# XiandaGuo/OpenStereo

Measured on NVIDIA H100. Metric: stereo_pairs_per_sec_gwcnet_256x512_d192, higher is better.
Workload: dtype f32

## Files before the change

### include/openstereo_b200.h

```cpp
#ifndef OPENSTEREO_B200_H_
#define OPENSTEREO_B200_H_

#include <stddef.h>
#include <stdint.h>

#ifdef __cplusplus
extern "C" {
#endif

#define OSB_OK 0
#define OSB_EINVAL 1
#define OSB_ECUDA 2
#define OSB_EUNSUPPORTED 3

#define OSB_ACT_NONE 0
#define OSB_ACT_RELU 1
#define OSB_ACT_LEAKY 2
#define OSB_ACT_RELU6 3

typedef void* osb_stream_t;

int osb_abi_version(void);
const char* osb_last_error(void);
uint64_t osb_launch_count(void);
// ... 85 lines not shown
                            osb_stream_t stream);
int osb_conv3d_k3_s2_tc_cs_fwd(const float* x_ndhwc, const void* w_split, const float* scale, const float* shift, float* y, int B,
                               int Cin, int Cout, int D, int H, int W, int act, int ystride, osb_stream_t stream);
int osb_deconv3d_k4_tc_cs_fwd(const float* x_ndhwc, const void* w_split, const float* scale, const float* shift, float* y, int B,
                              int Cin, int Cout, int D, int H, int W, int act, int ystride, osb_stream_t stream);
int osb_conv1x1_ndhwc_cat_fwd(const float* x0, const float* x1, int C0, int C1, const float* w_packed, const float* scale,
                              const float* shift, float* y, long long voxels, int Cout, int act, osb_stream_t stream);
int osb_conv1x1_ndhwc_fwd(const float* x, const float* w_packed, const float* scale, const float* shift, float* y,
                          long long voxels, int Cin, int Cout, int act, osb_stream_t stream);
int osb_conv3d_k3_c1_ndhwc_fwd(const float* x_ndhwc, const float* w_taps, const float* scale, const float* shift, float* y, int B,
                               int Cin, int D, int H, int W, osb_stream_t stream);
int osb_conv2d_tc_kc(int Cin, int Cout, int W, int dilation);
int osb_conv2d_k3_tc_fwd(const float* x_nhwc, const void* w_split, const float* scale, const float* shift, const float* residual,
                         float* y, int B, int Cin, int Cout, int H, int W, int dilation, int act, int out_nhwc, int res_nhwc,
                         osb_stream_t stream);
int osb_gwc_volume_sum_fwd(const float* ref, const float* tgt, float* out, int B, int C, int H, int W, int D, int G,
                           osb_stream_t stream);
int osb_group_l2_normalize_fwd(const float* x, float* y, int B, int C, int H, int W, int G, float eps, osb_stream_t stream);
int osb_sub_volume_fwd(const float* left, const float* right, float* out, int B, int C, int H, int W, int D, osb_stream_t stream);
int osb_regression_values_fwd(const float* prob, const float* values, float* out, int B, int D, int H, int W, osb_stream_t stream);

int osb_warped_concat_volume_fwd(const float* x, const float* y, const float* disp, float* out, int B, int C, int D, int H, int W,
                                 int mask_left, osb_stream_t stream);
int osb_warped_gwc_concat_volume_fwd(const float* xg, const float* yg, const float* xc, const float* yc, const float* disp,
                                     float* out, int B, int Cg, int G, int Cc, int D, int H, int W, osb_stream_t stream);

int osb_coex_regression_fwd(const float* cost, const float* spx, float* out, int B, int D, int h, int w, int top_k, int spx_is_logits,
                            osb_stream_t stream);
int osb_nearest_resize3d_fwd(const float* x, float* y, int N, int Di, int Hi, int Wi, int Do, int Ho, int Wo, osb_stream_t stream);

// ... 34 lines not shown
```

### openstereo_b200/_lib.py

```python
import ctypes
import os

_PKG = os.path.dirname(os.path.abspath(__file__))
LIB_PATH = os.path.join(_PKG, "lib", "libopenstereo_b200.so")

_f32p = ctypes.c_void_p
_i = ctypes.c_int
_f = ctypes.c_float
_s = ctypes.c_void_p

SIGNATURES = {
    "osb_gwc_volume_fwd": [_f32p, _f32p, _f32p, _i, _i, _i, _i, _i, _i, _s],
    "osb_concat_volume_fwd": [_f32p, _f32p, _f32p, _i, _i, _i, _i, _i, _i, _s],
    "osb_gwc_concat_volume_fwd": [_f32p, _f32p, _f32p, _f32p, _f32p, _i, _i, _i, _i, _i, _i, _i, _s],
    "osb_corr_volume_fwd": [_f32p, _f32p, _f32p, _i, _i, _i, _i, _i, _s],
    "osb_softargmin_fwd": [_f32p, _f32p, _i, _i, _i, _i, _f, _f, _f, _i, _s],
    "osb_upsample_softargmin_fwd": [_f32p, _f32p, _i, _i, _i, _i, _i, _i, _i, _i, _s],
    "osb_epe_partial_fwd": [_f32p, _f32p, _f32p, _i, _i, _f, _s],
    "osb_conv3d_k3_bn_act_fwd": [_f32p] * 7 + [_i] * 8 + [_s],
    "osb_deconv3d_bn_act_fwd": [_f32p] * 6 + [_i] * 8 + [_s],
    "osb_conv3d_1x1_bn_act_fwd": [_f32p, _f32p, _i] + [_f32p] * 6 + [_i] * 8 + [_s],
    "osb_conv3d_tc_supported": [_i, _i, _i, _i],
    "osb_conv3d_tc_kc": [_i, _i, _i, _i],
    "osb_tc_general_width": [_i],
# ... 9 lines not shown
    "osb_deconv3d_k4_tc_supported": [_i, _i, _i],
    "osb_conv3d_k3_tc_cs_fwd": [_f32p] * 7 + [_i] * 8 + [_s],
    "osb_conv3d_k3_s2_tc_cs_fwd": [_f32p] * 5 + [_i] * 8 + [_s],
    "osb_deconv3d_k4_tc_cs_fwd": [_f32p] * 5 + [_i] * 8 + [_s],
    "osb_deconv3d_k4_tc_fwd": [_f32p] * 6 + [_i] * 10 + [_s],
    "osb_conv1x1_ndhwc_cat_fwd": [_f32p, _f32p, _i, _i, _f32p, _f32p, _f32p, _f32p, ctypes.c_longlong, _i, _i, _s],
    "osb_feature_att_gate_fwd": [_f32p] * 8 + [_i] * 7 + [_s],
    "osb_ncdhw_to_ndhwc_pad": [_f32p, _f32p, _i, _i, _i, _i, _i, _i, _s],
    "osb_conv1x1_ndhwc_fwd": [_f32p] * 5 + [ctypes.c_longlong, _i, _i, _i, _s],
    "osb_conv3d_k3_c1_ndhwc_fwd": [_f32p] * 5 + [_i] * 5 + [_s],
    "osb_avgpool_pairs_fwd": [_f32p, _f32p, ctypes.c_longlong, _i, ctypes.c_longlong, _s],
    "osb_geo_lookup_fwd": [_f32p] * 11 + [_i] * 8 + [_s],
    "osb_context_upsample_fwd": [_f32p] * 3 + [_i] * 4 + [_s],
    "osb_conv2d_tc_kc": [_i] * 4,
    "osb_conv2d_k3_tc_fwd": [_f32p] * 6 + [_i] * 9 + [_s],
    "osb_ncdhw_to_ndhwc": [_f32p, _f32p, _i, _i, _i, _i, _i, _s],
    "osb_gwc_volume_sum_fwd": [_f32p, _f32p, _f32p, _i, _i, _i, _i, _i, _i, _s],
    "osb_group_l2_normalize_fwd": [_f32p, _f32p, _i, _i, _i, _i, _i, _f, _s],
    "osb_sub_volume_fwd": [_f32p, _f32p, _f32p, _i, _i, _i, _i, _i, _s],
    "osb_regression_values_fwd": [_f32p, _f32p, _f32p, _i, _i, _i, _i, _s],
    "osb_gwc_volume_bwd": [_f32p] * 5 + [_i] * 7 + [_s],
    "osb_concat_volume_bwd": [_f32p] * 3 + [_i] * 6 + [_s],
    "osb_softargmin_bwd": [_f32p] * 3 + [_i] * 4 + [_f, _f, _f, _i, _s],
    "osb_dwconv2d_fwd": [_f32p] * 6 + [_i] * 8 + [_s],
    "osb_deconv2d_k3s2_fwd": [_f32p] * 6 + [_i] * 6 + [_s],
    "osb_upsample_softargmin_values_fwd": [_f32p] * 3 + [_i] * 8 + [_s],
    "osb_warped_concat_volume_fwd": [_f32p] * 4 + [_i] * 6 + [_s],
    "osb_warped_gwc_concat_volume_fwd": [_f32p] * 6 + [_i] * 7 + [_s],
    "osb_coex_regression_fwd": [_f32p] * 3 + [_i] * 6 + [_s],
    "osb_nearest_resize3d_fwd": [_f32p] * 2 + [_i] * 7 + [_s],
# ... 58 lines not shown
```

### openstereo_b200/csrc/conv3d_tc.cu

```cuda
#include <type_traits>

#include "tc_common.cuh"

namespace osb {

constexpr int TC_W = 128;
constexpr int TC_KC = 32;
constexpr int TC_TILES = TC_WGS;
constexpr int TC_ROWS = TC_TILES + 2;
constexpr int TC_STAGES = 4;
constexpr int TC_RAW = 2;
constexpr int TC_ROW_BYTES = TC_W * TC_KC * 4;

struct TcParams {
  CUtensorMap xmap;
  const float* x;
  const void* w;
  const float* scale;
  const float* shift;
  const float* residual;
  float* y;
  int B, D, H, Cin, Cout;
  int act;
  float kappa;
// ... 402 lines not shown
  unsigned int* flag = tc_overflow_flag();
  if (!flag) return OSB_ECUDA;
  const size_t vol = (size_t)D * H * W;
  dim3 grid((unsigned)((vol + 31) / 32), (C + 31) / 32, B);
  ncdhw_to_ndhwc_kernel<<<grid, 256, 0, (cudaStream_t)stream>>>(x, nullptr, C, C, vol, reinterpret_cast<uint16_t*>(y_split), flag);
  count_launch();
  return check_launch("ncdhw_to_ndhwc_kernel");
}

int osb_ncdhw_to_ndhwc(const float* x, float* y, int B, int C, int D, int H, int W, osb_stream_t stream) {
  return osb_ncdhw_to_ndhwc_pad(x, y, B, C, C, D, H, W, stream);
}

static int conv3d_k3_tc_impl(osb::TcArgs a, int dilation, osb_stream_t stream) {
  using namespace osb;
  const int kc = select_conv3d_tc(a.Cin, a.Cout, a.W, dilation, false, false).kc;
  OSB_REQUIRE(kc, "conv3d_k3_tc: unsupported shape Cin=%d Cout=%d W=%d dilation=%d", a.Cin, a.Cout, a.W, dilation);
  OSB_REQUIRE(!a.in_ncdhw || kc == 32, "conv3d_k3_tc: NCDHW input is served by the W = 128 kernel only");
  OSB_REQUIRE((!a.ystride && !a.gate) || kc == 16, "conv3d_k3_tc: a channel slice or gate needs the 16-channel-chunk kernels");
  OSB_REQUIRE(a.Cout > 16 || (!a.out_ndhwc && (!a.residual || !a.res_ndhwc)), "conv3d_k3_tc: Cout <= 16 writes (and adds) NCDHW tensors only");
  OSB_REQUIRE(!(a.in_split || a.out_split || a.res_split) || (kc == 32 && !a.ystride && !a.gate),
              "conv3d_k3_tc: split activations are served by the W = 128 kernel only");
  OSB_REQUIRE(!a.in_split || !a.in_ncdhw, "conv3d_k3_tc: an input is either NCDHW or split");
  OSB_REQUIRE((!a.out_split || a.out_ndhwc) && (!a.res_split || a.res_ndhwc), "conv3d_k3_tc: split tensors are channels-last");
  OSB_REQUIRE(!(a.out_split || a.res_split) || (a.out_ndhwc && (!a.residual || a.res_ndhwc)),
              "conv3d_k3_tc: a split output or residual needs a channels-last output and residual");
  const TcLaunch launch = select_conv3d_tc(a.Cin, a.Cout, a.W, dilation, a.gate != nullptr, a.slice()).launch;
  const int rc = check_tc_args("conv3d_k3_tc", a, launch);
  return rc != OSB_OK ? rc : launch(a, (cudaStream_t)stream);
}

int osb_conv3d_k3_tc_fwd(const float* x_ndhwc, const void* w_split, const float* scale, const float* shift,
                         const float* residual, float* y, int B, int Cin, int Cout, int D, int H, int W, int act,
                         int out_ndhwc, int res_ndhwc, osb_stream_t stream) {
  return conv3d_k3_tc_impl({x_ndhwc, w_split, scale, shift, residual, nullptr, y, B, Cin, Cout, D, H, W, act, out_ndhwc, res_ndhwc, 0, 0,
                            Cout}, 1, stream);
}

int osb_conv3d_k3_tc_gate_fwd(const float* x_ndhwc, const void* w_split, const float* scale, const float* shift,
                              const float* residual, const float* gate_nhwc, float* y, int B, int Cin, int Cout, int D, int H, int W,
                              int act, osb_stream_t stream) {
// ... 4 lines not shown

int osb_conv3d_k3_tc_cs_fwd(const float* x_ndhwc, const void* w_split, const float* scale, const float* shift, const float* residual,
                            const float* gate_nhwc, float* y, int B, int Cin, int Cout, int D, int H, int W, int act, int ystride,
                            osb_stream_t stream) {
  return conv3d_k3_tc_impl({x_ndhwc, w_split, scale, shift, residual, gate_nhwc, y, B, Cin, Cout, D, H, W, act, 1, 1, 0, ystride, Cout},
                           1, stream);
}

int osb_conv3d_k3_tc_ncdhw_fwd(const float* x_ncdhw, const void* w_split, const float* scale, const float* shift,
                               const float* residual, float* y, int B, int Cin, int Cout, int D, int H, int W, int act,
                               int out_ndhwc, int res_ndhwc, osb_stream_t stream) {
  return conv3d_k3_tc_impl({x_ncdhw, w_split, scale, shift, residual, nullptr, y, B, Cin, Cout, D, H, W, act, out_ndhwc, res_ndhwc, 1, 0,
                            Cout}, 1, stream);
}

int osb_conv3d_k3_tc_split_fwd(const float* x, const void* w_split, const float* scale, const float* shift, const float* residual,
                               float* y, int B, int Cin, int Cout, int D, int H, int W, int act, int in_layout, int out_layout,
                               int res_layout, osb_stream_t stream) {
  auto known = [](int l) { return l == OSB_LAYOUT_NCDHW || l == OSB_LAYOUT_NDHWC || l == OSB_LAYOUT_SPLIT; };
  OSB_REQUIRE(known(in_layout) && known(out_layout) && known(res_layout), "conv3d_k3_tc_split: unknown layout");
  osb::TcArgs a{x, w_split, scale, shift, residual, nullptr, y, B, Cin, Cout, D, H, W, act, out_layout != OSB_LAYOUT_NCDHW, res_layout != OSB_LAYOUT_NCDHW,
                in_layout == OSB_LAYOUT_NCDHW, 0, Cout};
  a.in_split = in_layout == OSB_LAYOUT_SPLIT, a.out_split = out_layout == OSB_LAYOUT_SPLIT, a.res_split = res_layout == OSB_LAYOUT_SPLIT;
  return conv3d_k3_tc_impl(a, 1, stream);
}

int osb_conv2d_tc_kc(int Cin, int Cout, int W, int dilation) { return osb::select_conv3d_tc(Cin, Cout, W, dilation, false, false).kc; }

int osb_conv2d_k3_tc_fwd(const float* x_nhwc, const void* w_split, const float* scale, const float* shift, const float* residual,
                         float* y, int B, int Cin, int Cout, int H, int W, int dilation, int act, int out_nhwc, int res_nhwc,
                         osb_stream_t stream) {
  return conv3d_k3_tc_impl({x_nhwc, w_split, scale, shift, residual, nullptr, y, B, Cin, Cout, 1, H, W, act, out_nhwc, res_nhwc, 0, 0,
                            Cout}, dilation, stream);
}
}
```

### openstereo_b200/csrc/conv3d_tcg.cu

```cuda
#include "tc_common.cuh"

namespace osb {

struct TcgParams {
  const float* x;
  const void* w;
  const float* scale;
  const float* shift;
  const float* residual;
  const float* gate;
  float* y;
  int B, D, H, Cin;
  int act;
  float kappa;
  unsigned int* overflow;
  int out_ndhwc, res_ndhwc;
  int items, hblocks;
  int Wr, ctiles;
  int ystride;
};

template <int COUT, int KC, int W, int TILES, int DIL = 1, bool GW = false>
struct TcgCfg {
  static_assert(!GW || W == 128, "general-width tiles are 128-column segments of one image row");
  static constexpr int HALO = GW ? DIL : 0;
  static constexpr int CSTEP = 128 - 2 * HALO;
  static_assert(DIL == 1 || (W == 128 && DIL == 2 && COUT >= 64), "dilation 2 is instantiated for full-width rows only");
  static constexpr int R = 128 / W;
  static constexpr int ROWB = KC * 4;
  static constexpr int UNIT_BYTES = 128 * ROWB;
  static constexpr int N3 = 3 * COUT;
  static constexpr int G = 32;
  static constexpr int NG = COUT / G;
  static constexpr int NG3 = 3 * G;
  static constexpr int B_SLICE = N3 * ROWB;
  static constexpr int B_SUB = NG3 * ROWB;
  static constexpr int NT = TC_WGS * TILES;
  static constexpr int TS = R * DIL;
  static constexpr int HSPAN = NT * TS;
  __host__ __device__ static constexpr int row0(int hb) { return (hb / DIL) * HSPAN + (hb % DIL) * R; }
  __host__ static int hblocks(int H) { return DIL * ((H + HSPAN - 1) / HSPAN); }
  static constexpr int NLW = 4;
  static constexpr int XCHG_FLOATS = 2 * frag_xchg_floats<G, DIL>();
// ... 25 lines not shown
    return n;
  }
  static constexpr int NU = units_per_phase();
  static constexpr int unit_s(int j) {
    int k = 0;
    for (int s = S_FIRST; s <= S_LAST; ++s)
      if (used(s)) {
        if (k == j) return s;
        ++k;
      }
    return S_LAST;
  }
};

template <int COUT, int KC, int W, int TILES, int DIL = 1, bool GW = false, bool GATE = false>
__global__ void __launch_bounds__(TcgCfg<COUT, KC, W, TILES, DIL, GW>::THREADS, 1) conv3d_tcg_kernel(const TcgParams p) {
  using C = TcgCfg<COUT, KC, W, TILES, DIL, GW>;
  extern __shared__ __align__(1024) uint8_t smem_raw[];
  uint8_t* smem = reinterpret_cast<uint8_t*>((reinterpret_cast<uintptr_t>(smem_raw) + 1023) & ~static_cast<uintptr_t>(1023));
  uint8_t* a_buf = smem + C::A_OFF;
  uint8_t* b_buf = smem + C::B_OFF;
  uint64_t* bars = reinterpret_cast<uint64_t*>(smem + C::BAR_OFF);
  uint64_t* a_ready = bars;
  uint64_t* a_empty = a_ready + C::STAGES;
  uint64_t* b_full = a_empty + C::STAGES;
  uint64_t* b_empty = b_full + TC_BSLOTS * 3;
  float* xchg = reinterpret_cast<float*>(smem + C::BAR_OFF + 1024);
  float* tiles = xchg + TC_WGS * C::XCHG_FLOATS;
  float* s_scale = tiles + 4 * TC_WGS * FRAG_TP_FLOATS;
  float* s_shift = s_scale + COUT;

  const int warp = threadIdx.x >> 5, lane = threadIdx.x & 31;
  const int nchunk = p.Cin / KC;
  const int Wp = GW ? p.Wr : W;
  const int YS = (W < 32 && p.ystride) ? p.ystride : COUT;
  const int ctiles = GW ? p.ctiles : 1;

  if (threadIdx.x == 0) {
    for (int s = 0; s < C::STAGES; ++s) {
      mbar_init(&a_ready[s], 32);
      mbar_init(&a_empty[s], 4 * TC_WGS);
    }
    for (int k = 0; k < TC_BSLOTS * 3; ++k) {
      mbar_init(&b_full[k], 1);
      mbar_init(&b_empty[k], 4 * TC_WGS);
    }
    fence_mbar_init();
  }
  for (int c = threadIdx.x; c < COUT; c += blockDim.x) {
    s_scale[c] = p.scale ? p.scale[c] : 1.f;
    s_shift[c] = p.shift ? p.shift[c] : 0.f;
  }
  __syncthreads();

  if (warp < 4 * TC_WGS) {
// ... 16 lines not shown
      auto tile_row = [&](int m, int& h, int& col) {
        h = C::row0(hb) + wg * C::TS + m / W;
        col = GW ? ct * C::CSTEP - C::HALO + m : m % W;
        return h < p.H && (!GW || (m >= C::HALO && m < 128 - C::HALO && col < Wp));
      };
      {
        int h, col;
        if (tile_row(q * 32 + lane, h, col)) {
          const ptrdiff_t vox = (((ptrdiff_t)b * p.D + d) * p.H + h) * Wp + col;
          if (p.residual && p.res_ndhwc) asm volatile("prefetch.global.L2 [%0];" ::"l"(p.residual + vox * YS + cg));
          if (GATE && p.gate) asm volatile("prefetch.global.L2 [%0];" ::"l"(p.gate + (((ptrdiff_t)b * p.H + h) * Wp + col) * YS + cg));
        }
      }
      float acc[2][C::NG3 / 2];
      uint32_t accum = 0;
      for (int kd = 0; kd < 3; ++kd) {
        const int din = d + kd - 1;
        if (din < 0 || din >= p.D) continue;
        for (int ch = 0; ch < nchunk; ++ch, ++phc) {
#pragma unroll
          for (int s = C::S_FIRST; s <= C::S_LAST; ++s) {
            if (!C::used(s)) continue;
            const uint32_t slot = unitc % C::STAGES, par = (unitc / C::STAGES) & 1;
            mbar_wait(&a_ready[slot], par);
            const uint64_t da0 = dbase | (uint64_t)((smem_u32(a_buf + slot * C::UNIT_BYTES) & 0x3FFFF) >> 4);
#pragma unroll
            for (int kh = 0; kh < 3; ++kh) {
              if (C::tile_of(s, kh) != wg) continue;
              const uint32_t bslot = (phc & 1) * 3 + kh;
              mbar_wait(&b_full[bslot], (phc >> 1) & 1);
              const uint64_t db0 = dbase | (uint64_t)(b16 + (bslot * C::B_SUB) / 16);
              wg_fence();
#pragma unroll
              for (int ks = 0; ks < C::KSTEPS; ++ks)
                wg_mma_split<C::NG3>(acc, da0 + TcK<KC>::A_KSTEP * ks, A_HALF, TcK<KC>::A_LO, db0 + 2 * ks, TcK<KC>::B_LO, ks > 0 ? 1u : accum);
              wg_commit();
              wg_wait_all();
              accum = 1;
              wg_release(&b_empty[bslot], lane);
            }
            wg_release(&a_empty[slot], lane);
            ++unitc;
          }
        }
      }
      const float corr = 1.f + p.kappa * (float)(((d > 0) + 1 + (d + 1 < p.D)) * nchunk * 3 * C::KSTEPS * 3);
      frag_unshift<C::G, DIL, W>(acc, xchg + (exc & 1) * (C::XCHG_FLOATS / 2), q, lane, corr, bar_xchg);
      ++exc;
      const size_t plane = (size_t)p.D * p.H * Wp;
      auto rows = [&](int m, ptrdiff_t& yo, ptrdiff_t& ro, ptrdiff_t& go) {
        int h, col;
        const bool ok = tile_row(m, h, col);
        const ptrdiff_t vox = (((ptrdiff_t)b * p.D + d) * p.H + h) * Wp + col;
        const ptrdiff_t ncdhw = (ptrdiff_t)b * COUT * plane + ((ptrdiff_t)d * p.H + h) * Wp + col;
        yo = p.out_ndhwc ? vox * YS : ncdhw;
        ro = p.res_ndhwc ? vox * YS : ncdhw;
        go = (((ptrdiff_t)b * p.H + h) * Wp + col) * YS;
        return ok;
      };
      frag_epilogue<C::G>(acc, lane, q, tiles + warp * FRAG_TP_FLOATS, s_scale + cg, s_shift + cg, p.act, p.y + (p.out_ndhwc ? (size_t)cg : cg * plane),
                          p.out_ndhwc ? 1 : plane, p.residual ? p.residual + (p.res_ndhwc ? (size_t)cg : cg * plane) : nullptr,
                          p.res_ndhwc ? 1 : plane, (GATE && p.gate) ? p.gate + cg : nullptr, rows, C::G);
    }
  }
  else if (warp < 4 * TC_WGS + C::NLW) {
    setmaxnreg_dec<TC_LOADER_REGS>();
    const int lw = warp - 4 * TC_WGS;
    static_assert(KC == 16, "lane_voxel / unit-row mapping below is written for 64-byte operand rows");
    constexpr int CPR = KC / 4;
    constexpr int VPL = 32 / CPR;
    constexpr int NLD = 128 / VPL;
    static_assert(W % VPL == 0, "a load instruction must not straddle image rows");
    const int v0 = lane_voxel<KC>(lane), c = lane % CPR;
    float amax = 0.f;
    uint32_t ubase = 0;
    int first = lw;
    auto fill = [&](const float* base, size_t rstride, size_t cstride, int h_first, int h_step, uint32_t u, int col0) {
      float4 v[NLD];
#pragma unroll
      for (int j = 0; j < NLD; ++j) {
        const int hin = h_first + h_step * ((VPL * j) / W);
// ... 59 lines not shown
                         C::G * C::ROWB, &b_full[slot]);
            }
          }
        }
      }
    }
    __syncwarp();
  }
}

template <int COUT, int KC, int W, int TILES, int DIL = 1, bool GW = false, bool GATE = false>
static int launch_tcg(const TcArgs& a, cudaStream_t stream) {
  using C = TcgCfg<COUT, KC, W, TILES, DIL, GW>;
  TcgParams p{};
  p.gate = a.gate, p.ystride = a.ystride;
  p.hblocks = C::hblocks(a.H);
  p.Wr = GW ? a.W : W;
  p.ctiles = GW ? (a.W + C::CSTEP - 1) / C::CSTEP : 1;
  static const std::string variant = tc_variant_name("tcg<%d,%d,%d,%d,%d,%d,%d>", COUT, KC, W, TILES, DIL, (int)GW, (int)GATE);
  return launch_persistent<conv3d_tcg_kernel<COUT, KC, W, TILES, DIL, GW, GATE>>(
      a, p, (long long)a.B * a.D * p.hblocks * p.ctiles * C::NG, C::SMEM, variant.c_str(), stream);
}

TcRoute select_conv3d_tc(int Cin, int Cout, int W, int dilation, bool gate, bool slice) {
  if (dilation == 1 && W == 128 && Cin % 32 == 0 && Cin >= 32 && !gate && !slice) {
    if (Cout == 32) return {launch_tc<32>, 32};
    if (Cout >= 1 && Cout <= 16) return {launch_tc<16>, 32};
  }
  if (Cin % 16 != 0 || Cin < 16) return {};
  if (dilation == 2)
    return (W == 128 && Cout == 128 && !gate && !slice) ? TcRoute{launch_tcg<128, 16, 128, 1, 2>, 16} : TcRoute{};
  if (dilation != 1) return {};
  if (W == 16) {
    if (Cout == 96) return {launch_tcg<96, 16, 16, 1, 1, false, true>, 16};
    if (Cout == 64) return {launch_tcg<64, 16, 16, 1, 1, false, true>, 16};
    return {};
  }
  if (slice) return {};
  if (gate) {
    if (W == 64 && Cout == 64) return {launch_tcg<64, 16, 64, 1, 1, false, true>, 16};
    if (W == 32 && Cout == 96) return {launch_tcg<96, 16, 32, 1, 1, false, true>, 16};
    return {};
  }
  if (W == 64 && Cout == 64) return {launch_tcg<64, 16, 64, 1>, 16};
  if (W == 32 && Cout == 64) return {launch_tcg<64, 16, 32, 1>, 16};
  if (W == 32 && Cout == 128) return {launch_tcg<128, 16, 32, 1>, 16};
  if (W == 32 && Cout == 96) return {launch_tcg<96, 16, 32, 1>, 16};
  if (W == 128 && Cout == 64) return {launch_tcg<64, 16, 128, 1>, 16};
  if (W == 128 && Cout == 128) return {launch_tcg<128, 16, 128, 1>, 16};
  if (!osb_tc_general_width(W)) return {};
  if (Cout == 32) return {launch_tcg<32, 16, 128, 1, 1, true>, 16};
  if (Cout == 64) return {launch_tcg<64, 16, 128, 1, 1, true>, 16};
  if (Cout == 128) return {launch_tcg<128, 16, 128, 1, 1, true>, 16};
  return {};
}

}
```

### openstereo_b200/csrc/tc_common.cuh

```cuda
#pragma once
#include "common.cuh"

namespace osb {

__device__ __forceinline__ void mbar_wait_relaxed(uint64_t* bar, uint32_t parity) {
  uint32_t done;
  for (;;) {
    asm volatile(
        "{\n.reg .pred p;\nmbarrier.try_wait.parity.shared::cta.b64 p, [%1], %2;\nselp.u32 %0, 1, 0, p;\n}\n"
        : "=r"(done)
        : "r"(smem_u32(bar)), "r"(parity)
        : "memory");
    if (done) return;
    __nanosleep(64);
  }
}
__device__ __forceinline__ void mbar_arrive(uint64_t* bar) {
  asm volatile("mbarrier.arrive.shared::cta.b64 _, [%0];" ::"r"(smem_u32(bar)) : "memory");
}
__device__ __forceinline__ uint64_t desc_sw128_base() {
  uint64_t d = 0;
  d |= (uint64_t)1 << 16;
  d |= (uint64_t)(1024 >> 4) << 32;
  d |= (uint64_t)1 << 62;
// ... 50 lines not shown
}

template <>
__device__ __forceinline__ void wgmma_f16<128>(float (&d)[64], uint64_t da, uint64_t db, uint32_t accumulate) {
  asm volatile(
      "{\n.reg .pred p;\nsetp.ne.b32 p, %66, 0;\n"
      "wgmma.mma_async.sync.aligned.m64n128k16.f32.f16.f16 {%0, %1, %2, %3, %4, %5, %6, %7, %8, %9, %10, %11, %12, %13, %14, %15, %16, %17, %18, %19, %20, %21, %22, %23, %24, %25, %26, %27, %28, %29, %30, %31, %32, %33, %34, %35, %36, %37, %38, %39, %40, %41, %42, %43, %44, %45, %46, %47, %48, %49, %50, %51, %52, %53, %54, %55, %56, %57, %58, %59, %60, %61, %62, %63}, %64, %65, p, 1, 1, 0, 0;\n}\n"
      : "+f"(d[0]), "+f"(d[1]), "+f"(d[2]), "+f"(d[3]), "+f"(d[4]), "+f"(d[5]), "+f"(d[6]), "+f"(d[7]), "+f"(d[8]), "+f"(d[9]), "+f"(d[10]), "+f"(d[11]), "+f"(d[12]), "+f"(d[13]), "+f"(d[14]), "+f"(d[15]), "+f"(d[16]), "+f"(d[17]), "+f"(d[18]), "+f"(d[19]), "+f"(d[20]), "+f"(d[21]), "+f"(d[22]), "+f"(d[23]), "+f"(d[24]), "+f"(d[25]), "+f"(d[26]), "+f"(d[27]), "+f"(d[28]), "+f"(d[29]), "+f"(d[30]), "+f"(d[31]), "+f"(d[32]), "+f"(d[33]), "+f"(d[34]), "+f"(d[35]), "+f"(d[36]), "+f"(d[37]), "+f"(d[38]), "+f"(d[39]), "+f"(d[40]), "+f"(d[41]), "+f"(d[42]), "+f"(d[43]), "+f"(d[44]), "+f"(d[45]), "+f"(d[46]), "+f"(d[47]), "+f"(d[48]), "+f"(d[49]), "+f"(d[50]), "+f"(d[51]), "+f"(d[52]), "+f"(d[53]), "+f"(d[54]), "+f"(d[55]), "+f"(d[56]), "+f"(d[57]), "+f"(d[58]), "+f"(d[59]), "+f"(d[60]), "+f"(d[61]), "+f"(d[62]), "+f"(d[63])
      : "l"(da), "l"(db), "r"(accumulate)
      : "memory");
}

__device__ __forceinline__ void wg_fence() { asm volatile("wgmma.fence.sync.aligned;" ::: "memory"); }
__device__ __forceinline__ void wg_commit() { asm volatile("wgmma.commit_group.sync.aligned;" ::: "memory"); }
__device__ __forceinline__ void wg_wait_all() { asm volatile("wgmma.wait_group.sync.aligned 0;" ::: "memory"); }

template <int N>
__device__ __forceinline__ void wg_mma_split(float (&acc)[2][N / 2], uint64_t da, uint32_t a_half, uint32_t a_lo, uint64_t db,
                                             uint32_t b_lo, uint32_t accumulate) {
#pragma unroll
  for (int h = 0; h < 2; ++h) {
    wgmma_f16<N>(acc[h], da + h * a_half + a_lo, db, accumulate);
    wgmma_f16<N>(acc[h], da + h * a_half, db + b_lo, 1);
    wgmma_f16<N>(acc[h], da + h * a_half, db, 1);
  }
}
__device__ __forceinline__ void wg_release(uint64_t* bar, int lane) {
  if (lane == 0) mbar_arrive(bar);
}
template <int N>
// ... 93 lines not shown

constexpr int SPLIT_GRANULE = 16;
__device__ __forceinline__ int split_index(int c) { return (c / SPLIT_GRANULE) * 2 * SPLIT_GRANULE + c % SPLIT_GRANULE; }
__device__ __forceinline__ void split_store4(uint16_t* vox, int c, const float4 v, float& amax) {
  uint2 hi, lo;
  f16_split4(v, hi, lo, amax);
  *reinterpret_cast<uint2*>(vox + split_index(c)) = hi;
  *reinterpret_cast<uint2*>(vox + split_index(c) + SPLIT_GRANULE) = lo;
}
__device__ __forceinline__ float4 split_load4(const uint16_t* vox, int c) {
  const uint2 hi = __ldg(reinterpret_cast<const uint2*>(vox + split_index(c)));
  const uint2 lo = __ldg(reinterpret_cast<const uint2*>(vox + split_index(c) + SPLIT_GRANULE));
  const float2 h01 = f16x2_to_float2(hi.x), h23 = f16x2_to_float2(hi.y), l01 = f16x2_to_float2(lo.x), l23 = f16x2_to_float2(lo.y);
  constexpr float inv = 1.f / TC_ACT_SCALE;
  return make_float4((h01.x + l01.x) * inv, (h01.y + l01.y) * inv, (h23.x + l23.x) * inv, (h23.y + l23.y) * inv);
}

template <int KC>
__device__ __forceinline__ void stage_f16_split(uint8_t* tile, int row, int q, const float4 v, float& amax) {
  uint2 hi, lo;
  f16_split4(v, hi, lo, amax);
  const int sub = (q & 1) << 3, chunk = 4 * (q >> 2) + ((q >> 1) & 1);
  *reinterpret_cast<uint2*>(tile + swz_offset<KC>(row, chunk) + sub) = hi;
  *reinterpret_cast<uint2*>(tile + swz_offset<KC>(row, chunk + 2) + sub) = lo;
}
template <int KC>
__device__ __forceinline__ int lane_voxel(int lane) {
  if constexpr (KC == 32) return (((lane >> 3) & 1) << 1) | (lane >> 4);
  else return ((lane >> 2) & 1) | (((lane >> 3) & 1) << 2) | ((lane >> 4) << 1);
}
// ... 134 lines not shown
  }
#pragma unroll
  for (int h = 0; h < 2; ++h) {
    float2 rv[G / 8][2], gv[G / 8][2];
#pragma unroll
    for (int j = 0; j < G / 8; ++j)
#pragma unroll
      for (int rh = 0; rh < 2; ++rh) {
        const int c = 8 * j + c0;
        ptrdiff_t yo, ro, go;
        const bool live = rows(64 * h + 16 * wq + l4 + 8 * rh, yo, ro, go);
        rv[j][rh] = make_float2(0.f, 0.f);
        gv[j][rh] = make_float2(1.f, 1.f);
        if (res) {
          if (rcs == 1) {
            if (live) rv[j][rh] = __ldg(reinterpret_cast<const float2*>(res + ro + c));
          } else {
            if (live && c < nch) rv[j][rh].x = __ldg(res + ro + (size_t)c * rcs);
            if (live && c + 1 < nch) rv[j][rh].y = __ldg(res + ro + (size_t)(c + 1) * rcs);
          }
        }
        if (gate && live) gv[j][rh] = __ldg(reinterpret_cast<const float2*>(gate + go + c));
      }
#pragma unroll
    for (int j = 0; j < G / 8; ++j) {
      const int c = 8 * j + c0;
      const float2 a = *reinterpret_cast<const float2*>(sc + c);
      const float2 b = *reinterpret_cast<const float2*>(sh + c);
#pragma unroll
      for (int rh = 0; rh < 2; ++rh) {
        ptrdiff_t yo, ro, go;
// ... 136 lines not shown
  const cudaError_t e = cudaGetLastError();
  if (e != cudaSuccess) {
    cudaFuncAttributes fa{};
    (void)cudaFuncGetAttributes(&fa, KERNEL);
    set_error("%s: launch failed: %s (threads %d, kernel maxThreadsPerBlock %d, regs %d, static smem %zu, dynamic smem %zu, "
              "max dynamic %d)", variant, cudaGetErrorString(e), TC_WG_THREADS, fa.maxThreadsPerBlock, fa.numRegs,
              fa.sharedSizeBytes, smem, fa.maxDynamicSharedSizeBytes);
    return OSB_ECUDA;
  }
  return OSB_OK;
}

struct TcRoute {
  TcLaunch launch;
  int kc;
};
TcRoute select_conv3d_tc(int Cin, int Cout, int W, int dilation, bool gate, bool slice);
template <int COUT>
int launch_tc(const TcArgs& a, cudaStream_t stream);

}
```

### openstereo_b200/host_models.py

```python
import torch
import torch.nn as nn
import torch.nn.functional as F

from . import aggregation as _agg
from . import ops
from .aggregation import GwcAggregation, PSMAggregation


USE_TC_BACKBONE = True


def _cfg_get(cfgs, key, default=None):
    if isinstance(cfgs, dict):
        return cfgs.get(key, default)
    return getattr(cfgs, key, default)


def _cb(cin, cout, k, stride, pad, dilation, bias=False):
    return nn.Sequential(nn.Conv2d(cin, cout, kernel_size=k, stride=stride, padding=dilation if dilation > 1 else pad,
                                   dilation=dilation, bias=bias), nn.BatchNorm2d(cout))


def _front_tc_ok(net, x):
    return (getattr(net, "_osb_folded", False) and x.is_cuda and x.dim() == 4 and x.shape[2] == 2 * ops.TC_WIDTH and x.shape[3] % 2 == 0
# ... 2 lines not shown

def _front_tc(net, x):
    convs = [m for m in net.firstconv.modules() if isinstance(m, nn.Conv2d)]
    blocks = list(net.layer1.children())
    y = F.relu(convs[0](x))
    t = y.permute(0, 3, 2, 1).contiguous()
    t = _tc2d(net, convs[2], _tc2d(net, convs[1], t, ops.ACT_RELU, transpose=True), ops.ACT_RELU, transpose=True)
    for i, blk in enumerate(blocks):
        c1, c2 = _block_convs(blk)
        assert blk.downsample is None
        t = _tc2d(net, c2, _tc2d(net, c1, t, ops.ACT_RELU, transpose=True), ops.ACT_NONE, residual=t, last=(i == len(blocks) - 1),
                  transpose=True)
    return t.transpose(2, 3).contiguous()


def _tc2d(net, conv, t, act, residual=None, last=False, transpose=False):
    cache = net.__dict__.setdefault("_osb_tc2d", {})
    dil = conv.dilation[0]
    if id(conv) not in cache:
        assert conv.kernel_size == (3, 3) and conv.stride == (1, 1) and conv.padding == (dil, dil) and conv.dilation == (dil, dil)
        w5 = torch.zeros(conv.out_channels, conv.in_channels, 3, 3, 3, dtype=torch.float32, device=conv.weight.device)
        w2 = conv.weight.detach().float()
        w5[:, :, 1] = w2.transpose(2, 3) if transpose else w2
        kc = ops.conv2d_tc_kc(conv.in_channels, conv.out_channels, ops.TC_WIDTH, dil)
        cache[id(conv)] = (ops.pack_tc_weight(w5, kc), None if conv.bias is None else conv.bias.detach().float().contiguous())
    wp, bias = cache[id(conv)]
    return ops.conv2d_k3_tc(t, wp, None, bias, residual, act, dil, out_nhwc=not last, res_nhwc=True)


def _block_convs(blk):
    c1 = [m for m in blk.conv1.modules() if isinstance(m, nn.Conv2d)][0]
    c2 = [m for m in blk.conv2.modules() if isinstance(m, nn.Conv2d)][0]
    return c1, c2


def _block_tc_ok(blk, c):
    if blk.downsample is not None:
        return False
    c1, c2 = _block_convs(blk)
    dil = c1.dilation[0]
    return all(cv.kernel_size == (3, 3) and cv.stride == (1, 1) and cv.dilation == (dil, dil) and cv.padding == (dil, dil)
               and cv.in_channels == c and cv.out_channels == c for cv in (c1, c2)) and ops.conv2d_tc_kc(c, c, ops.TC_WIDTH, dil) != 0


def _stage_tc(net, stage, x):
    blocks = list(stage.children())
    usable = getattr(net, "_osb_folded", False) and x.is_cuda and x.dtype == torch.float32 and _agg.USE_TENSOR_CORES and USE_TC_BACKBONE
    y, rest = x, blocks
    if not (usable and x.shape[3] == ops.TC_WIDTH and _block_tc_ok(blocks[0], x.shape[1])):
        y, rest = blocks[0](x), blocks[1:]
    c = y.shape[1]
    if not (usable and rest and y.shape[3] == ops.TC_WIDTH and all(_block_tc_ok(b, c) for b in rest)):
        for b in rest:
            y = b(y)
        return y
    t = ops.to_ndhwc(y.unsqueeze(2).contiguous()).squeeze(1)
    for i, b in enumerate(rest):
        c1, c2 = _block_convs(b)
        t = _tc2d(net, c2, _tc2d(net, c1, t, ops.ACT_RELU), ops.ACT_NONE, residual=t, last=(i == len(rest) - 1))
    return t


def _lastconv_tc_ok(net, x):
    convs = [m for m in net.lastconv.modules() if isinstance(m, nn.Conv2d)]
    return (getattr(net, "_osb_folded", False) and x.is_cuda and x.dtype == torch.float32 and _agg.USE_TENSOR_CORES and USE_TC_BACKBONE
            and x.shape[3] == ops.TC_WIDTH and len(convs) == 2 and convs[0].kernel_size == (3, 3) and convs[0].stride == (1, 1)
            and convs[0].dilation == (1, 1) and convs[0].padding == (1, 1) and convs[1].kernel_size == (1, 1)
            and ops.conv2d_tc_kc(convs[0].in_channels, convs[0].out_channels, ops.TC_WIDTH, 1) != 0)


def _lastconv_tc(net, x):
    convs = [m for m in net.lastconv.modules() if isinstance(m, nn.Conv2d)]
    t = ops.to_ndhwc(x.unsqueeze(2).contiguous()).squeeze(1)
    return convs[1](_tc2d(net, convs[0], t, ops.ACT_RELU, last=True))


def gwc_extract(net, x):
    x = _front_tc(net, x) if _front_tc_ok(net, x) else net.layer1(net.firstconv(x))
    l2 = _stage_tc(net, net.layer2, x)
    l3 = _stage_tc(net, net.layer3, l2)
    l4 = _stage_tc(net, net.layer4, l3)
    gwc = torch.cat((l2, l3, l4), dim=1)
    out = {"gwc_feature": gwc}
    if net.concat_feature:
        out["concat_feature"] = _lastconv_tc(net, gwc) if _lastconv_tc_ok(net, gwc) else net.lastconv(gwc)
    return out


# ... 299 lines not shown
```

### openstereo_b200/ops.py

```python
import math

import torch

from . import _lib

ACT_NONE, ACT_RELU, ACT_LEAKY, ACT_RELU6 = 0, 1, 2, 3
TC_WIDTH = 128
TC_KC = 32


_LAUNCH_DEVICE = [None]


def _stream(t):
    _LAUNCH_DEVICE[0] = t.device.index
    return torch.cuda.current_stream(t.device).cuda_stream


def _same_device(*tensors):
    devs = {t.device for t in tensors if t is not None}
    if len(devs) > 1:
        raise RuntimeError("openstereo_b200: operands live on different devices: %s" % sorted(str(d) for d in devs))


# ... 882 lines not shown

def context_upsample(disp_low, up_weights, scale_factor=4):
    assert disp_low.is_cuda and disp_low.dim() == 4 and disp_low.shape[1] == 1
    b, _, h, w = disp_low.shape
    assert tuple(up_weights.shape) == (b, 9, h * scale_factor, w * scale_factor)
    disp_low, up_weights = disp_low.contiguous().float(), up_weights.contiguous().float()
    out = torch.empty((b, h * scale_factor, w * scale_factor), dtype=torch.float32, device=disp_low.device)
    _call("osb_context_upsample_fwd", disp_low.data_ptr(), up_weights.data_ptr(), out.data_ptr(), b, h, w, scale_factor, _stream(out))
    return out


def conv2d_tc_kc(cin, cout, w, dilation=1):
    return int(_lib.lib.osb_conv2d_tc_kc(int(cin), int(cout), int(w), int(dilation)))


def conv2d_k3_tc(x_nhwc, w_split, scale=None, shift=None, residual=None, act=ACT_NONE, dilation=1, out_nhwc=True, res_nhwc=True):
    assert x_nhwc.is_cuda and x_nhwc.dtype == torch.float32 and x_nhwc.is_contiguous() and x_nhwc.dim() == 4
    b, h, w, cin = x_nhwc.shape
    cout = w_split.cout
    kc = conv2d_tc_kc(cin, cout, w, dilation)
    assert kc
    wptr, scale = _tc_args(w_split, cin, kc, scale)
    y = torch.empty((b, h, w, cout) if out_nhwc else (b, cout, h, w), dtype=torch.float32, device=x_nhwc.device)
    if residual is not None:
        assert residual.is_contiguous() and residual.numel() == y.numel()
    _call("osb_conv2d_k3_tc_fwd", x_nhwc.data_ptr(), wptr, _ptr(scale), _ptr(shift), _ptr(residual), y.data_ptr(), b, cin,
          cout, h, w, dilation, act, int(out_nhwc), int(res_nhwc), _stream(y))
    return y
```

Measured before the change: 297.7.

## Carry split fp16 activations through 2D feature-stage conv chains with TMA loads

Extends the tensor-core 2D conv path so that 128-channel feature stages keep activations in the split hi/lo fp16 layout between convolutions. The W=128, Cout=128 kernel gains a TMA loader for split inputs and can read split residuals. The MMA loop now waits on the previous wgmma group instead of all groups, deferring buffer release by one step. The intent is to cut fp32 activation traffic and per-thread gather loads, and to overlap consecutive MMAs. The cost is more layout conversions and more complex buffer-release ordering.

New measurement: 302.5, median of 6. 1.6% higher.

```diff
diff --git a/include/openstereo_b200.h b/include/openstereo_b200.h
--- a/include/openstereo_b200.h
+++ b/include/openstereo_b200.h
@@ -123,6 +123,9 @@
 int osb_conv2d_k3_tc_fwd(const float* x_nhwc, const void* w_split, const float* scale, const float* shift, const float* residual,
                          float* y, int B, int Cin, int Cout, int H, int W, int dilation, int act, int out_nhwc, int res_nhwc,
                          osb_stream_t stream);
+int osb_conv2d_k3_tc_split_fwd(const float* x, const void* w_split, const float* scale, const float* shift, const float* residual,
+                               float* y, int B, int Cin, int Cout, int H, int W, int dilation, int act, int in_layout, int out_layout,
+                               int res_layout, osb_stream_t stream);
 int osb_gwc_volume_sum_fwd(const float* ref, const float* tgt, float* out, int B, int C, int H, int W, int D, int G,
                            osb_stream_t stream);
 int osb_group_l2_normalize_fwd(const float* x, float* y, int B, int C, int H, int W, int G, float eps, osb_stream_t stream);
diff --git a/openstereo_b200/_lib.py b/openstereo_b200/_lib.py
--- a/openstereo_b200/_lib.py
+++ b/openstereo_b200/_lib.py
@@ -47,6 +47,7 @@
     "osb_context_upsample_fwd": [_f32p] * 3 + [_i] * 4 + [_s],
     "osb_conv2d_tc_kc": [_i] * 4,
     "osb_conv2d_k3_tc_fwd": [_f32p] * 6 + [_i] * 9 + [_s],
+    "osb_conv2d_k3_tc_split_fwd": [_f32p] * 6 + [_i] * 10 + [_s],
     "osb_ncdhw_to_ndhwc": [_f32p, _f32p, _i, _i, _i, _i, _i, _s],
     "osb_gwc_volume_sum_fwd": [_f32p, _f32p, _f32p, _i, _i, _i, _i, _i, _i, _s],
     "osb_group_l2_normalize_fwd": [_f32p, _f32p, _i, _i, _i, _i, _i, _f, _s],
diff --git a/openstereo_b200/csrc/conv3d_tc.cu b/openstereo_b200/csrc/conv3d_tc.cu
--- a/openstereo_b200/csrc/conv3d_tc.cu
+++ b/openstereo_b200/csrc/conv3d_tc.cu
@@ -440,17 +440,17 @@
 
 static int conv3d_k3_tc_impl(osb::TcArgs a, int dilation, osb_stream_t stream) {
   using namespace osb;
-  const int kc = select_conv3d_tc(a.Cin, a.Cout, a.W, dilation, false, false).kc;
+  const TcRoute shape = select_conv3d_tc(a.Cin, a.Cout, a.W, dilation, false, false);
+  const int kc = shape.kc;
   OSB_REQUIRE(kc, "conv3d_k3_tc: unsupported shape Cin=%d Cout=%d W=%d dilation=%d", a.Cin, a.Cout, a.W, dilation);
   OSB_REQUIRE(!a.in_ncdhw || kc == 32, "conv3d_k3_tc: NCDHW input is served by the W = 128 kernel only");
   OSB_REQUIRE((!a.ystride && !a.gate) || kc == 16, "conv3d_k3_tc: a channel slice or gate needs the 16-channel-chunk kernels");
   OSB_REQUIRE(a.Cout > 16 || (!a.out_ndhwc && (!a.residual || !a.res_ndhwc)), "conv3d_k3_tc: Cout <= 16 writes (and adds) NCDHW tensors only");
-  OSB_REQUIRE(!(a.in_split || a.out_split || a.res_split) || (kc == 32 && !a.ystride && !a.gate),
-              "conv3d_k3_tc: split activations are served by the W = 128 kernel only");
+  OSB_REQUIRE(!(a.in_split || a.out_split || a.res_split) || (shape.split && !a.ystride && !a.gate),
+              "conv3d_k3_tc: split activations are served by the W = 128 kernel only (whole rows, no gate, no channel slice)");
   OSB_REQUIRE(!a.in_split || !a.in_ncdhw, "conv3d_k3_tc: an input is either NCDHW or split");
   OSB_REQUIRE((!a.out_split || a.out_ndhwc) && (!a.res_split || a.res_ndhwc), "conv3d_k3_tc: split tensors are channels-last");
-  OSB_REQUIRE(!(a.out_split || a.res_split) || (a.out_ndhwc && (!a.residual || a.res_ndhwc)),
-              "conv3d_k3_tc: a split output or residual needs a channels-last output and residual");
+  OSB_REQUIRE(!a.out_split || !a.residual || a.res_ndhwc, "conv3d_k3_tc: a split output needs a channels-last residual");
   const TcLaunch launch = select_conv3d_tc(a.Cin, a.Cout, a.W, dilation, a.gate != nullptr, a.slice()).launch;
   const int rc = check_tc_args("conv3d_k3_tc", a, launch);
   return rc != OSB_OK ? rc : launch(a, (cudaStream_t)stream);
@@ -485,15 +485,19 @@
                             Cout}, 1, stream);
 }
 
+static int conv3d_k3_tc_layouts(osb::TcArgs a, int dilation, int in_layout, int out_layout, int res_layout, osb_stream_t stream) {
+  auto known = [](int l) { return l == OSB_LAYOUT_NCDHW || l == OSB_LAYOUT_NDHWC || l == OSB_LAYOUT_SPLIT; };
+  OSB_REQUIRE(known(in_layout) && known(out_layout) && known(res_layout), "conv3d_k3_tc_split: unknown layout");
+  a.out_ndhwc = out_layout != OSB_LAYOUT_NCDHW, a.res_ndhwc = res_layout != OSB_LAYOUT_NCDHW, a.in_ncdhw = in_layout == OSB_LAYOUT_NCDHW;
+  a.in_split = in_layout == OSB_LAYOUT_SPLIT, a.out_split = out_layout == OSB_LAYOUT_SPLIT, a.res_split = res_layout == OSB_LAYOUT_SPLIT;
+  return conv3d_k3_tc_impl(a, dilation, stream);
+}
+
 int osb_conv3d_k3_tc_split_fwd(const float* x, const void* w_split, const float* scale, const float* shift, const float* residual,
                                float* y, int B, int Cin, int Cout, int D, int H, int W, int act, int in_layout, int out_layout,
                                int res_layout, osb_stream_t stream) {
-  auto known = [](int l) { return l == OSB_LAYOUT_NCDHW || l == OSB_LAYOUT_NDHWC || l == OSB_LAYOUT_SPLIT; };
-  OSB_REQUIRE(known(in_layout) && known(out_layout) && known(res_layout), "conv3d_k3_tc_split: unknown layout");
-  osb::TcArgs a{x, w_split, scale, shift, residual, nullptr, y, B, Cin, Cout, D, H, W, act, out_layout != OSB_LAYOUT_NCDHW, res_layout != OSB_LAYOUT_NCDHW,
-                in_layout == OSB_LAYOUT_NCDHW, 0, Cout};
-  a.in_split = in_layout == OSB_LAYOUT_SPLIT, a.out_split = out_layout == OSB_LAYOUT_SPLIT, a.res_split = res_layout == OSB_LAYOUT_SPLIT;
-  return conv3d_k3_tc_impl(a, 1, stream);
+  return conv3d_k3_tc_layouts({x, w_split, scale, shift, residual, nullptr, y, B, Cin, Cout, D, H, W, act, 0, 0, 0, 0, Cout}, 1, in_layout,
+                              out_layout, res_layout, stream);
 }
 
 int osb_conv2d_tc_kc(int Cin, int Cout, int W, int dilation) { return osb::select_conv3d_tc(Cin, Cout, W, dilation, false, false).kc; }
@@ -504,4 +508,11 @@
   return conv3d_k3_tc_impl({x_nhwc, w_split, scale, shift, residual, nullptr, y, B, Cin, Cout, 1, H, W, act, out_nhwc, res_nhwc, 0, 0,
                             Cout}, dilation, stream);
 }
-}
+
+int osb_conv2d_k3_tc_split_fwd(const float* x, const void* w_split, const float* scale, const float* shift, const float* residual,
+                               float* y, int B, int Cin, int Cout, int H, int W, int dilation, int act, int in_layout, int out_layout,
+                               int res_layout, osb_stream_t stream) {
+  return conv3d_k3_tc_layouts({x, w_split, scale, shift, residual, nullptr, y, B, Cin, Cout, 1, H, W, act, 0, 0, 0, 0, Cout}, dilation,
+                              in_layout, out_layout, res_layout, stream);
+}
+}
diff --git a/openstereo_b200/csrc/conv3d_tcg.cu b/openstereo_b200/csrc/conv3d_tcg.cu
--- a/openstereo_b200/csrc/conv3d_tcg.cu
+++ b/openstereo_b200/csrc/conv3d_tcg.cu
@@ -3,6 +3,7 @@
 namespace osb {
 
 struct TcgParams {
+  CUtensorMap xmap;
   const float* x;
   const void* w;
   const float* scale;
@@ -15,6 +16,7 @@
   float kappa;
   unsigned int* overflow;
   int out_ndhwc, res_ndhwc;
+  int in_split, out_split, res_split;
   int items, hblocks;
   int Wr, ctiles;
   int ystride;
@@ -27,6 +29,7 @@
   static constexpr int CSTEP = 128 - 2 * HALO;
   static_assert(DIL == 1 || (W == 128 && DIL == 2 && COUT >= 64), "dilation 2 is instantiated for full-width rows only");
   static constexpr int R = 128 / W;
+  static constexpr bool SPLIT = W == 128 && !GW && COUT == 128;
   static constexpr int ROWB = KC * 4;
   static constexpr int UNIT_BYTES = 128 * ROWB;
   static constexpr int N3 = 3 * COUT;
@@ -82,7 +85,7 @@
 };
 
 template <int COUT, int KC, int W, int TILES, int DIL = 1, bool GW = false, bool GATE = false>
-__global__ void __launch_bounds__(TcgCfg<COUT, KC, W, TILES, DIL, GW>::THREADS, 1) conv3d_tcg_kernel(const TcgParams p) {
+__global__ void __launch_bounds__(TcgCfg<COUT, KC, W, TILES, DIL, GW>::THREADS, 1) conv3d_tcg_kernel(const __grid_constant__ TcgParams p) {
   using C = TcgCfg<COUT, KC, W, TILES, DIL, GW>;
   extern __shared__ __align__(1024) uint8_t smem_raw[];
   uint8_t* smem = reinterpret_cast<uint8_t*>((reinterpret_cast<uintptr_t>(smem_raw) + 1023) & ~static_cast<uintptr_t>(1023));
@@ -106,7 +109,7 @@
 
   if (threadIdx.x == 0) {
     for (int s = 0; s < C::STAGES; ++s) {
-      mbar_init(&a_ready[s], 32);
+      mbar_init(&a_ready[s], (C::SPLIT && p.in_split) ? 1 : 32);
       mbar_init(&a_empty[s], 4 * TC_WGS);
     }
     for (int k = 0; k < TC_BSLOTS * 3; ++k) {
@@ -153,6 +156,7 @@
       }
       float acc[2][C::NG3 / 2];
       uint32_t accum = 0;
+      int pend_a = -1, pend_b = 0;
       for (int kd = 0; kd < 3; ++kd) {
         const int din = d + kd - 1;
         if (din < 0 || din >= p.D) continue;
@@ -163,6 +167,7 @@
             const uint32_t slot = unitc % C::STAGES, par = (unitc / C::STAGES) & 1;
             mbar_wait(&a_ready[slot], par);
             const uint64_t da0 = dbase | (uint64_t)((smem_u32(a_buf + slot * C::UNIT_BYTES) & 0x3FFFF) >> 4);
+            bool mine = false;
 #pragma unroll
             for (int kh = 0; kh < 3; ++kh) {
               if (C::tile_of(s, kh) != wg) continue;
@@ -174,14 +179,24 @@
               for (int ks = 0; ks < C::KSTEPS; ++ks)
                 wg_mma_split<C::NG3>(acc, da0 + TcK<KC>::A_KSTEP * ks, A_HALF, TcK<KC>::A_LO, db0 + 2 * ks, TcK<KC>::B_LO, ks > 0 ? 1u : accum);
               wg_commit();
-              wg_wait_all();
+              wg_wait_prev();
               accum = 1;
-              wg_release(&b_empty[bslot], lane);
+              if (pend_a >= 0) {
+                wg_release(&b_empty[pend_b], lane);
+                wg_release(&a_empty[pend_a], lane);
+              }
+              pend_a = (int)slot, pend_b = (int)bslot;
+              mine = true;
             }
-            wg_release(&a_empty[slot], lane);
+            if (!mine) wg_release(&a_empty[slot], lane);
             ++unitc;
           }
         }
+      }
+      wg_wait_all();
+      if (pend_a >= 0) {
+        wg_release(&b_empty[pend_b], lane);
+        wg_release(&a_empty[pend_a], lane);
       }
       const float corr = 1.f + p.kappa * (float)(((d > 0) + 1 + (d + 1 < p.D)) * nchunk * 3 * C::KSTEPS * 3);
       frag_unshift<C::G, DIL, W>(acc, xchg + (exc & 1) * (C::XCHG_FLOATS / 2), q, lane, corr, bar_xchg);
@@ -199,11 +214,42 @@
       };
       frag_epilogue<C::G>(acc, lane, q, tiles + warp * FRAG_TP_FLOATS, s_scale + cg, s_shift + cg, p.act, p.y + (p.out_ndhwc ? (size_t)cg : cg * plane),
                           p.out_ndhwc ? 1 : plane, p.residual ? p.residual + (p.res_ndhwc ? (size_t)cg : cg * plane) : nullptr,
-                          p.res_ndhwc ? 1 : plane, (GATE && p.gate) ? p.gate + cg : nullptr, rows, C::G);
+                          p.res_ndhwc ? 1 : plane, (GATE && p.gate) ? p.gate + cg : nullptr, rows, C::G, C::SPLIT && p.out_split,
+                          C::SPLIT && p.res_split, p.overflow);
     }
   }
   else if (warp < 4 * TC_WGS + C::NLW) {
     setmaxnreg_dec<TC_LOADER_REGS>();
+    if constexpr (C::SPLIT) {
+      if (p.in_split) {
+        if (warp == 4 * TC_WGS && elect_one()) {
+          uint32_t unitc = 0;
+          for (int it = blockIdx.x; it < p.items; it += gridDim.x) {
+            const int it0 = it / C::NG;
+            const int h0 = C::row0(it0 % p.hblocks);
+            const int d = (it0 / p.hblocks) % p.D;
+            const int b = it0 / (p.hblocks * p.D);
+            for (int kd = 0; kd < 3; ++kd) {
+              const int din = d + kd - 1;
+              if (din < 0 || din >= p.D) continue;
+              for (int ch = 0; ch < nchunk; ++ch) {
+#pragma unroll
+                for (int s = C::S_FIRST; s <= C::S_LAST; ++s) {
+                  if (!C::used(s)) continue;
+                  const uint32_t slot = unitc % C::STAGES, ph = (unitc / C::STAGES) & 1;
+                  mbar_wait_relaxed(&a_empty[slot], ph ^ 1);
+                  mbar_arrive_expect_tx(&a_ready[slot], C::UNIT_BYTES);
+                  tma_load_4d(a_buf + slot * C::UNIT_BYTES, &p.xmap, &a_ready[slot], 2 * KC * ch, 0, h0 + s, b * p.D + din);
+                  ++unitc;
+                }
+              }
+            }
+          }
+        }
+        __syncwarp();
+        return;
+      }
+    }
     const int lw = warp - 4 * TC_WGS;
     static_assert(KC == 16, "lane_voxel / unit-row mapping below is written for 64-byte operand rows");
     constexpr int CPR = KC / 4;
@@ -293,6 +339,8 @@
   using C = TcgCfg<COUT, KC, W, TILES, DIL, GW>;
   TcgParams p{};
   p.gate = a.gate, p.ystride = a.ystride;
+  p.in_split = a.in_split, p.out_split = a.out_split, p.res_split = a.res_split;
+  if (a.in_split && !make_tensor_map_split(&p.xmap, a.x, a.Cin, W, a.H, a.B * a.D, KC)) return OSB_ECUDA;
   p.hblocks = C::hblocks(a.H);
   p.Wr = GW ? a.W : W;
   p.ctiles = GW ? (a.W + C::CSTEP - 1) / C::CSTEP : 1;
@@ -303,12 +351,12 @@
 
 TcRoute select_conv3d_tc(int Cin, int Cout, int W, int dilation, bool gate, bool slice) {
   if (dilation == 1 && W == 128 && Cin % 32 == 0 && Cin >= 32 && !gate && !slice) {
-    if (Cout == 32) return {launch_tc<32>, 32};
-    if (Cout >= 1 && Cout <= 16) return {launch_tc<16>, 32};
+    if (Cout == 32) return {launch_tc<32>, 32, true};
+    if (Cout >= 1 && Cout <= 16) return {launch_tc<16>, 32, true};
   }
   if (Cin % 16 != 0 || Cin < 16) return {};
   if (dilation == 2)
-    return (W == 128 && Cout == 128 && !gate && !slice) ? TcRoute{launch_tcg<128, 16, 128, 1, 2>, 16} : TcRoute{};
+    return (W == 128 && Cout == 128 && !gate && !slice) ? TcRoute{launch_tcg<128, 16, 128, 1, 2>, 16, true} : TcRoute{};
   if (dilation != 1) return {};
   if (W == 16) {
     if (Cout == 96) return {launch_tcg<96, 16, 16, 1, 1, false, true>, 16};
@@ -326,7 +374,7 @@
   if (W == 32 && Cout == 128) return {launch_tcg<128, 16, 32, 1>, 16};
   if (W == 32 && Cout == 96) return {launch_tcg<96, 16, 32, 1>, 16};
   if (W == 128 && Cout == 64) return {launch_tcg<64, 16, 128, 1>, 16};
-  if (W == 128 && Cout == 128) return {launch_tcg<128, 16, 128, 1>, 16};
+  if (W == 128 && Cout == 128) return {launch_tcg<128, 16, 128, 1>, 16, true};
   if (!osb_tc_general_width(W)) return {};
   if (Cout == 32) return {launch_tcg<32, 16, 128, 1, 1, true>, 16};
   if (Cout == 64) return {launch_tcg<64, 16, 128, 1, 1, true>, 16};
diff --git a/openstereo_b200/csrc/tc_common.cuh b/openstereo_b200/csrc/tc_common.cuh
--- a/openstereo_b200/csrc/tc_common.cuh
+++ b/openstereo_b200/csrc/tc_common.cuh
@@ -88,6 +88,7 @@
 __device__ __forceinline__ void wg_fence() { asm volatile("wgmma.fence.sync.aligned;" ::: "memory"); }
 __device__ __forceinline__ void wg_commit() { asm volatile("wgmma.commit_group.sync.aligned;" ::: "memory"); }
 __device__ __forceinline__ void wg_wait_all() { asm volatile("wgmma.wait_group.sync.aligned 0;" ::: "memory"); }
+__device__ __forceinline__ void wg_wait_prev() { asm volatile("wgmma.wait_group.sync.aligned 1;" ::: "memory"); }
 
 template <int N>
 __device__ __forceinline__ void wg_mma_split(float (&acc)[2][N / 2], uint64_t da, uint32_t a_half, uint32_t a_lo, uint64_t db,
@@ -211,6 +212,12 @@
   const float2 h01 = f16x2_to_float2(hi.x), h23 = f16x2_to_float2(hi.y), l01 = f16x2_to_float2(lo.x), l23 = f16x2_to_float2(lo.y);
   constexpr float inv = 1.f / TC_ACT_SCALE;
   return make_float4((h01.x + l01.x) * inv, (h01.y + l01.y) * inv, (h23.x + l23.x) * inv, (h23.y + l23.y) * inv);
+}
+__device__ __forceinline__ float2 split_load2(const uint16_t* vox, int c) {
+  const float2 h = f16x2_to_float2(__ldg(reinterpret_cast<const uint32_t*>(vox + split_index(c))));
+  const float2 l = f16x2_to_float2(__ldg(reinterpret_cast<const uint32_t*>(vox + split_index(c) + SPLIT_GRANULE)));
+  constexpr float inv = 1.f / TC_ACT_SCALE;
+  return make_float2((h.x + l.x) * inv, (h.y + l.y) * inv);
 }
 
 template <int KC>
@@ -375,7 +382,9 @@
         gv[j][rh] = make_float2(1.f, 1.f);
         if (res) {
           if (rcs == 1) {
-            if (live) rv[j][rh] = __ldg(reinterpret_cast<const float2*>(res + ro + c));
+            if (live)
+              rv[j][rh] = res_split ? split_load2(reinterpret_cast<const uint16_t*>(res + ro), c)
+                                    : __ldg(reinterpret_cast<const float2*>(res + ro + c));
           } else {
             if (live && c < nch) rv[j][rh].x = __ldg(res + ro + (size_t)c * rcs);
             if (live && c + 1 < nch) rv[j][rh].y = __ldg(res + ro + (size_t)(c + 1) * rcs);
@@ -542,6 +551,7 @@
 struct TcRoute {
   TcLaunch launch;
   int kc;
+  bool split;
 };
 TcRoute select_conv3d_tc(int Cin, int Cout, int W, int dilation, bool gate, bool slice);
 template <int COUT>
diff --git a/openstereo_b200/host_models.py b/openstereo_b200/host_models.py
--- a/openstereo_b200/host_models.py
+++ b/openstereo_b200/host_models.py
@@ -40,7 +40,11 @@
     return t.transpose(2, 3).contiguous()
 
 
-def _tc2d(net, conv, t, act, residual=None, last=False, transpose=False):
+def _split_chain(c):
+    return c == 128
+
+
+def _tc2d(net, conv, t, act, residual=None, last=False, transpose=False, split=False):
     cache = net.__dict__.setdefault("_osb_tc2d", {})
     dil = conv.dilation[0]
     if id(conv) not in cache:
@@ -51,7 +55,7 @@
         kc = ops.conv2d_tc_kc(conv.in_channels, conv.out_channels, ops.TC_WIDTH, dil)
         cache[id(conv)] = (ops.pack_tc_weight(w5, kc), None if conv.bias is None else conv.bias.detach().float().contiguous())
     wp, bias = cache[id(conv)]
-    return ops.conv2d_k3_tc(t, wp, None, bias, residual, act, dil, out_nhwc=not last, res_nhwc=True)
+    return ops.conv2d_k3_tc(t, wp, None, bias, residual, act, dil, out_nhwc=not last, res_nhwc=True, out_split=split and not last)
 
 
 def _block_convs(blk):
@@ -80,10 +84,11 @@
         for b in rest:
             y = b(y)
         return y
-    t = ops.to_ndhwc(y.unsqueeze(2).contiguous()).squeeze(1)
+    split = _split_chain(c)
+    t = (ops.to_split if split else ops.to_ndhwc)(y.unsqueeze(2).contiguous()).squeeze(1)
     for i, b in enumerate(rest):
         c1, c2 = _block_convs(b)
-        t = _tc2d(net, c2, _tc2d(net, c1, t, ops.ACT_RELU), ops.ACT_NONE, residual=t, last=(i == len(rest) - 1))
+        t = _tc2d(net, c2, _tc2d(net, c1, t, ops.ACT_RELU, split=split), ops.ACT_NONE, residual=t, last=(i == len(rest) - 1), split=split)
     return t
 
 
@@ -97,7 +102,8 @@
 
 def _lastconv_tc(net, x):
     convs = [m for m in net.lastconv.modules() if isinstance(m, nn.Conv2d)]
-    t = ops.to_ndhwc(x.unsqueeze(2).contiguous()).squeeze(1)
+    split = _split_chain(convs[0].out_channels)
+    t = (ops.to_split if split else ops.to_ndhwc)(x.unsqueeze(2).contiguous()).squeeze(1)
     return convs[1](_tc2d(net, convs[0], t, ops.ACT_RELU, last=True))
 
 
diff --git a/openstereo_b200/ops.py b/openstereo_b200/ops.py
--- a/openstereo_b200/ops.py
+++ b/openstereo_b200/ops.py
@@ -920,13 +920,33 @@
     return int(_lib.lib.osb_conv2d_tc_kc(int(cin), int(cout), int(w), int(dilation)))
 
 
-def conv2d_k3_tc(x_nhwc, w_split, scale=None, shift=None, residual=None, act=ACT_NONE, dilation=1, out_nhwc=True, res_nhwc=True):
-    assert x_nhwc.is_cuda and x_nhwc.dtype == torch.float32 and x_nhwc.is_contiguous() and x_nhwc.dim() == 4
+def conv2d_k3_tc(x_nhwc, w_split, scale=None, shift=None, residual=None, act=ACT_NONE, dilation=1, out_nhwc=True, res_nhwc=True,
+                 out_split=False):
+    assert x_nhwc.is_cuda and x_nhwc.dtype in (torch.float32, torch.float16) and x_nhwc.is_contiguous() and x_nhwc.dim() == 4
+    in_split = is_split(x_nhwc.unsqueeze(1))
     b, h, w, cin = x_nhwc.shape
     cout = w_split.cout
+    if in_split:
+        cin = w_split.data.shape[1] * w_split.kc
+        if x_nhwc.shape[3] != 2 * cin:
+            raise ValueError("conv2d_k3_tc: an fp16 input is read as split activations (ops.to_split), 2 * Cin = %d entries per "
+                             "voxel for this weight; got %d" % (2 * cin, x_nhwc.shape[3]))
     kc = conv2d_tc_kc(cin, cout, w, dilation)
     assert kc
     wptr, scale = _tc_args(w_split, cin, kc, scale)
+    res_split = residual is not None and is_split(residual.unsqueeze(1))
+    if in_split or out_split or res_split:
+        assert out_nhwc or not out_split
+        if residual is not None:
+            want = (b, h, w, 2 * cout if res_split else cout) if res_nhwc else (b, cout, h, w)
+            assert tuple(residual.shape) == want and residual.is_contiguous() and (res_split or residual.dtype == torch.float32)
+        shape = (b, h, w, 2 * cout if out_split else cout) if out_nhwc else (b, cout, h, w)
+        y = torch.empty(shape, dtype=torch.float16 if out_split else torch.float32, device=x_nhwc.device)
+        layout = lambda split, nhwc: LAYOUT_SPLIT if split else (LAYOUT_NDHWC if nhwc else LAYOUT_NCDHW)
+        _call("osb_conv2d_k3_tc_split_fwd", x_nhwc.data_ptr(), wptr, _ptr(scale), _ptr(shift), _ptr(residual), y.data_ptr(), b, cin,
+              cout, h, w, dilation, act, layout(in_split, True), layout(out_split, out_nhwc), layout(res_split, res_nhwc), _stream(y),
+              profile_as="osb_conv2d_k3_tc_fwd")
+        return y
     y = torch.empty((b, h, w, cout) if out_nhwc else (b, cout, h, w), dtype=torch.float32, device=x_nhwc.device)
     if residual is not None:
         assert residual.is_contiguous() and residual.numel() == y.numel()
```
